# PJLab-ADG/neuralsim

Hardware: NVIDIA H100
Metric: Mrays/sec fwd+bwd (higher is better)
Workload: dtype f16

## Files before the change

### neuralsim_b200/csrc/fused_tc.cu

```cuda
#include "fused_tc_common.cuh"

namespace nsb {

constexpr int kSdfCtasPerSM = 4, kSdfPackCtasPerSM = 5;

template <int MODE>
__global__ void __launch_bounds__(kTile, MODE == 2 ? kSdfPackCtasPerSM : 0)
k_fused_sdf_tc(const PLMeta m, const __half *__restrict__ grid, const DecoderDevTC dec, const float *__restrict__ x,
               const float *__restrict__ rays_o, const float *__restrict__ rays_d, const int64_t *__restrict__ ridx,
               const float *__restrict__ t, int64_t n, int max_level, float *__restrict__ sdf, const int64_t *__restrict__ pack_infos,
               const int64_t *__restrict__ pack_ray, const int64_t *__restrict__ order, int64_t n_packs, const OccCollect oc,
               const int64_t *__restrict__ n_dev) {
    if (MODE == 2) n_packs = eff_n(n_packs, n_dev); else n = eff_n(n, n_dev);
    __shared__ __align__(128) uint8_t sA[kTile * NF * 2];
    __shared__ __align__(128) uint8_t sB[HW * NF * 2];
    __shared__ float sb1[HW], sW2[HW], srow[kTile];
    __shared__ float sb2;

    const int tid = threadIdx.x, warp = tid >> 5, lane = tid & 31;
    stage_W1(dec, sB, tid);
    stage_decoder_vectors(dec, sb1, sW2, &sb2, tid);
    tc::fence_async_smem();
    __syncthreads();
    const SdfTile ctx{m, grid, max_level, sA, tc::smem_u32(sA), tc::smem_u32(sB), srow, sb1, sW2, sb2, SoftplusK(dec.beta)};

    if (MODE == 2) {
        const int64_t n_groups = (n_packs + 31) / 32;
        for (int64_t g = blockIdx.x; g < n_groups; g += gridDim.x) {
            const int64_t slot = g * 32 + lane;
            int64_t first = 0, cnt = 0, ray = 0;
            if (slot < n_packs) {
                const int64_t p = order ? order[slot] : slot;
                first = pack_infos[2 * p]; cnt = pack_infos[2 * p + 1]; ray = pack_ray ? pack_ray[p] : p;
            }
            float o[3] = {0.f, 0.f, 0.f}, d[3] = {0.f, 0.f, 0.f};
            if (cnt > 0) {
#pragma unroll
                for (int q = 0; q < 3; ++q) { o[q] = rays_o[ray * 3 + q]; d[q] = rays_d[ray * 3 + q]; }
            }
            int max_n = (int)cnt;
#pragma unroll
            for (int s = 16; s > 0; s >>= 1) max_n = max(max_n, __shfl_xor_sync(0xffffffffu, max_n, s));
            for (int k0 = 0; k0 < max_n; k0 += kTile / 32) {
                const int k = k0 + warp;
                const bool valid = k < cnt;
                float xs[3] = {0.f, 0.f, 0.f};
                if (valid) {
                    const float tt = t[first + k];
#pragma unroll
                    for (int q = 0; q < 3; ++q) xs[q] = __fmaf_rn(d[q], tt, o[q]);
                }
#pragma unroll
                for (int q = 0; q < 3; ++q) xs[q] = to_table_space(xs[q]);
                const float v = sdf_of_tile(ctx, xs, tid);
                if (valid) {
                    sdf[first + k] = v;
                    if (oc.pcl) occ_collect_point(oc, xs, v);
                }
            }
        }
    } else {
        const int64_t n_tiles = (n + kTile - 1) / kTile;
        for (int64_t tile = blockIdx.x; tile < n_tiles; tile += gridDim.x) {
            const int64_t i = tile * kTile + tid;
            const bool valid = i < n;
            float xs[3];
            load_point(PointSrc{x, rays_o, rays_d, t, ridx}, MODE == 1, i, valid, xs);
            const float v = sdf_of_tile(ctx, xs, tid);
            if (valid) {
                sdf[i] = v;
                if (oc.pcl) occ_collect_point(oc, xs, v);
            }
        }
    }
}

constexpr int kSdfBwdCtasPerSM = 4;

template <bool FROM_RAYS, bool kXGrad>
__global__ void __launch_bounds__(kTile, kSdfBwdCtasPerSM)
k_sdf_bwd_tc(const PLMeta m, const __half *__restrict__ grid, const DecoderDevTC dec, const float *__restrict__ x,
             const float *__restrict__ rays_o, const float *__restrict__ rays_d, const int64_t *__restrict__ ridx,
             const float *__restrict__ t, const float *__restrict__ d_sdf, int64_t n, int max_level, float *__restrict__ d_grid,
             float *__restrict__ d_W1, float *__restrict__ d_b1, float *__restrict__ d_W2, float *__restrict__ d_b2,
             const int64_t *__restrict__ keep, const int64_t *__restrict__ n_dev, float *__restrict__ gx_out) {
    n = eff_n(n, n_dev);
    constexpr int NX = 40, GW = 128;
    constexpr int kS = tc::acc_stride(NF);
    extern __shared__ uint8_t dyn_smem[];
    uint8_t *tiles = reinterpret_cast<uint8_t *>((reinterpret_cast<uintptr_t>(dyn_smem) + 127) & ~uintptr_t(127));
    uint8_t *sA = tiles;
    uint8_t *sG = sA + kTile * NX * 2;
    uint8_t *sB = sG + kTile * GW * 2;
    uint8_t *sBT = sB + HW * NF * 2;
    float *stage = reinterpret_cast<float *>(sG);
    static_assert(kTile * kS * 4 <= kTile * GW * 2, "the staged dH rows must fit in G");
    __shared__ float sb1[HW], sW2[HW], sdd[kTile];
    __shared__ float sdb2;

    const int tid = threadIdx.x, lane = tid & 31;
    stage_W1(dec, sB, tid);
    stage_W1T(dec, sBT, tid);
    stage_decoder_vectors(dec, sb1, sW2, nullptr, tid);
    *reinterpret_cast<uint4 *>(sA + 4 * (kTile * 16) + tid * 16) = make_uint4(0x00003C00u, 0, 0, 0);
    float xacc[NX / 2], vacc[4];
#pragma unroll
    for (int k = 0; k < NX / 2; ++k) xacc[k] = 0.f;
#pragma unroll
    for (int k = 0; k < 4; ++k) vacc[k] = 0.f;
    if (tid == 0) sdb2 = 0.f;
    tc::fence_async_smem();
    __syncthreads();
    const uint32_t a_addr = tc::smem_u32(sA), g_addr = tc::smem_u32(sG), b_addr = tc::smem_u32(sB), bt_addr = tc::smem_u32(sBT);
    const SoftplusK spk(dec.beta);
    bool first_tile = true;

    const int64_t n_tiles = (n + kTile - 1) / kTile;
    for (int64_t tile = blockIdx.x; tile < n_tiles; tile += gridDim.x) {
        const int64_t i_ = tile * kTile + tid;
        const bool valid = i_ < n;
        const int64_t i = (valid && keep) ? keep[i_] : i_;
        float xs[3];
        load_point(PointSrc{x, rays_o, rays_d, t, ridx}, FROM_RAYS, i, valid, xs);
        const float dd = valid ? d_sdf[i] : 0.f;
        sdd[tid] = dd;
        gather_row_to_tile<kTile>(m, grid, xs, max_level, sA, tid);
        tc::fence_async_smem();
        __syncthreads();
        {
            float z[2][HW / 2];
            tc::mma_m128<HW, 0, 0, NF / 16>(z, tc::kmajor(a_addr, kTile), tc::kmajor(b_addr, HW), false);
#pragma unroll
            for (int h = 0; h < 2; ++h)
#pragma unroll
                for (int r = 0; r < 2; ++r) {
                    const int row = h * 64 + tc::frag_row(r);
                    const float d = sdd[row];
#pragma unroll
                    for (int c = 0; c < HW / 8; ++c) {
                        const int col = tc::frag_col(c);
                        float dz[2], da[2];
#pragma unroll
                        for (int j = 0; j < 2; ++j) {
                            const float zz = r16(z[h][4 * c + 2 * r + j] + sb1[col + j]);
                            float a, s;
                            softplus_as(zz, spk, a, s);
                            da[j] = d * r16(a);
                            dz[j] = d * sW2[col + j] * s;
                        }
                        tc::st_pair_f16(sG, tc::pair_off<kTile>(row, col), dz[0], dz[1]);
                        tc::st_pair_f16(sG, tc::pair_off<kTile>(row, HW + col), da[0], da[1]);
                    }
                }
        }
        tc::fence_async_smem();
        __syncthreads();
        float dh_fr[2][NF / 2];
        tc::mma_m128<NF, 0, 0, HW / 16>(dh_fr, tc::kmajor(g_addr, kTile), tc::kmajor(bt_addr, NF), false);
        tc::mma_m64<NX, 1, 1, kTile / 16>(xacc, tc::mnmajor(g_addr, kTile), tc::mnmajor(a_addr, kTile), true);
        tc::mma_m64<8, 1, 1, kTile / 16>(vacc, tc::mnmajor(g_addr + 8 * (kTile * 16), kTile), tc::mnmajor(a_addr + 4 * (kTile * 16), kTile), true);
        first_tile = false;
        const float dsum = warp_sum(dd);
        if (lane == 0 && dsum != 0.f) atomicAdd(&sdb2, dsum);
        __syncthreads();
        tc::frag_store<NF>(dh_fr, stage, kS, 0);
        __syncthreads();
        const bool active = valid && dd != 0.f;
        const bool warp_active = __any_sync(0xffffffffu, active);
        float gx[3] = {0.f, 0.f, 0.f};
#pragma unroll 1
        for (uint32_t g4 = 0; g4 * 4 < m.n_pseudo; ++g4) {
            float dh[8];
            tc::acc_ld8(stage, kS, tid, g4 * 8, dh);
            if (!warp_active) continue;
#pragma unroll
            for (uint32_t q = 0; q < 4; ++q) {
                const uint32_t p = g4 * 4 + q;
                if (p >= m.n_pseudo || (int)m.level[p] > max_level) continue;
                uint32_t cell[8];
                float w[8], a[8], b[8], fr[3], sc[3];
                if constexpr (kXGrad) level_cells3(m, p, xs, cell, w, fr, sc);
                else level_cells3(m, p, xs, cell, w);
                const float g0 = active ? dh[2 * q] : 0.f, g1 = active ? dh[2 * q + 1] : 0.f;
                if constexpr (kXGrad) level_input_grad(m, p, grid, cell, fr, sc, g0, g1, gx);
#pragma unroll
                for (int c = 0; c < 8; ++c) { a[c] = g0 * w[c]; b[c] = g1 * w[c]; }
                if (warp_merge_updates(cell_key3(m, p, xs), active, a, b, lane)) {
                    float2 *gp = level_grad_ptr(m, p, d_grid);
#pragma unroll
                    for (int c = 0; c < 8; ++c) red_add2(gp + cell[c], a[c], b[c]);
                }
            }
        }
        if constexpr (kXGrad) {
            if (valid) {
                float g[3];
#pragma unroll
                for (int d = 0; d < 3; ++d) g[d] = input_grad_to_net(gx[d]);
                const float tt = t[i];
                float4 *o = reinterpret_cast<float4 *>(gx_out + i_ * 8);
                o[0] = make_float4(g[0], g[1], g[2], __fmul_rn(tt, g[0]));
                o[1] = make_float4(__fmul_rn(tt, g[1]), __fmul_rn(tt, g[2]), 0.f, 0.f);
            }
        }
        __syncthreads();
    }
    if (!first_tile) {
#pragma unroll
        for (int r = 0; r < 2; ++r) {
            const int row = tc::frag_row(r);
            if (row >= dec.width) continue;
#pragma unroll
            for (int c = 0; c <= NF / 8; ++c)
#pragma unroll
                for (int j = 0; j < 2; ++j) {
                    const int col = tc::frag_col(c) + j;
                    if (col < dec.nh) atomicAdd(d_W1 + row * dec.nh + col, xacc[4 * c + 2 * r + j]);
                    else if (col == NF) atomicAdd(d_b1 + row, xacc[4 * c + 2 * r + j]);
                }
            if (tc::frag_col(0) == 0) atomicAdd(d_W2 + row, vacc[2 * r]);
        }
        if (tid == 0) atomicAdd(d_b2, sdb2);
    }
}

}

using namespace nsb;

extern "C" int nsb_fused_sdf_tc_launch(const nsb_lotd_meta *meta, const void *params_half, const nsb_sdf_decoder *dec, const float *x,
                                       const float *rays_o, const float *rays_d, const int64_t *ridx, const float *t, int64_t n,
                                       int32_t max_level, float *sdf, void *stream, int mode, const int64_t *pack_infos,
                                       const int64_t *pack_ray, const int64_t *pack_order, int64_t n_packs, const nsb_occ_collect *collect) {
    const DevCounts dn = take_counts();
    PLMeta m;
    DecoderDevTC d;
    if (int rc = make_decoder(meta, dec, &m, &d, "nsb_fused_sdf (tensor-core)")) return rc;
    cudaStream_t s = (cudaStream_t)stream;
    const int ml = max_level < 0 ? -1 : max_level;
    const __half *g = (const __half *)params_half;
    const OccCollect oc = occ_collect_of(collect);
    const unsigned tiles = persistent_grid((n + kTile - 1) / kTile, kSdfCtasPerSM);
    if (mode == 2 && require_ctas_per_sm(k_fused_sdf_tc<2>, kTile, 0, kSdfPackCtasPerSM, "nsb_fused_sdf (packs)")) return 2;
    if (mode == 2)
        k_fused_sdf_tc<2><<<persistent_grid((n_packs + 31) / 32, kSdfPackCtasPerSM), kTile, 0, s>>>(m, g, d, nullptr, rays_o, rays_d, nullptr, t, n, ml, sdf,
                                                                                                 pack_infos, pack_ray, pack_order, n_packs, oc, dn.a);
    else if (mode == 1)
        k_fused_sdf_tc<1><<<tiles, kTile, 0, s>>>(m, g, d, nullptr, rays_o, rays_d, ridx, t, n, ml, sdf, nullptr, nullptr, nullptr, 0, oc, dn.a);
    else
        k_fused_sdf_tc<0><<<tiles, kTile, 0, s>>>(m, g, d, x, nullptr, nullptr, nullptr, nullptr, n, ml, sdf, nullptr, nullptr, nullptr, 0, oc, dn.a);
    return check_launch("nsb_fused_sdf(tc)");
}

extern "C" int nsb_fused_sdf_bwd(const nsb_lotd_meta *meta, const void *params_half, const nsb_sdf_decoder *dec, const float *x,
                                 const float *rays_o, const float *rays_d, const int64_t *ridx, const float *t, const float *d_sdf,
                                 int64_t n, int32_t max_level, float *d_grid, float *d_W1, float *d_b1, float *d_W2, float *d_b2,
                                 void *stream) {
    return nsb_fused_sdf_bwd_indexed(meta, params_half, dec, x, rays_o, rays_d, ridx, t, d_sdf, nullptr, n, max_level, d_grid, d_W1, d_b1, d_W2, d_b2,
                                     stream);
}

template <bool kXGrad>
static int sdf_bwd(const char *who, const nsb_lotd_meta *meta, const void *params_half, const nsb_sdf_decoder *dec, const float *x, const float *rays_o,
                   const float *rays_d, const int64_t *ridx, const float *t, const float *d_sdf, const int64_t *keep, int64_t n, int32_t max_level,
                   float *d_grid, float *d_W1, float *d_b1, float *d_W2, float *d_b2, float *gx_scratch, const int64_t *ray_map, float *d_rays_o,
                   float *d_rays_d, void *stream) {
    const DevCounts dn = take_counts();
    if (n == 0) return 0;
    NSB_REQUIRE(meta && params_half && dec && d_sdf && d_grid && d_W1 && d_b1 && d_W2 && d_b2, "%s: NULL argument", who);
    NSB_REQUIRE(x || (rays_o && rays_d && t), "%s: need x or (rays_o, rays_d, t)", who);
    if (kXGrad) NSB_REQUIRE(!x && gx_scratch, "%s: ray gradients need the points as rays (x NULL) and gx_scratch", who);
    PLMeta m;
    DecoderDevTC d;
    if (int rc = make_decoder(meta, dec, &m, &d, who)) return rc;
    constexpr int kBwdSmem = (128 * 40 + 128 * 128 + 64 * 32 + 32 * 64) * 2 + 128;
    auto kern = x == nullptr ? k_sdf_bwd_tc<true, kXGrad> : k_sdf_bwd_tc<false, false>;
    opt_in_smem(kern, kBwdSmem);
    if (int rc = require_ctas_per_sm(kern, kTile, kBwdSmem, kSdfBwdCtasPerSM, who)) return rc;
    const unsigned grid = persistent_grid((n + kTile - 1) / kTile, kSdfBwdCtasPerSM);
    cudaStream_t s = (cudaStream_t)stream;
    const int ml = max_level < 0 ? -1 : max_level;
    kern<<<grid, kTile, kBwdSmem, s>>>(m, (const __half *)params_half, d, x, x ? nullptr : rays_o, x ? nullptr : rays_d, x ? nullptr : ridx,
                                       x ? nullptr : t, d_sdf, n, ml, d_grid, d_W1, d_b1, d_W2, d_b2, keep, dn.a, gx_scratch);
    if (int rc = check_launch(who)) return rc;
    if (kXGrad) {
        if (!d_rays_o && !d_rays_d) return 0;
        k_ray_row_sum<8><<<row_sum_blocks(n), 256, 0, s>>>(gx_scratch, ridx, keep, n, 6, ray_map, RowSumOut{{d_rays_o, d_rays_d, nullptr}, 3}, dn.a);
        return check_launch("nsb_fused_sdf_bwd_rays(ray sum)");
    }
    return 0;
}

extern "C" int nsb_fused_sdf_bwd_indexed(const nsb_lotd_meta *meta, const void *params_half, const nsb_sdf_decoder *dec, const float *x,
                                         const float *rays_o, const float *rays_d, const int64_t *ridx, const float *t, const float *d_sdf,
                                         const int64_t *keep, int64_t n, int32_t max_level, float *d_grid, float *d_W1, float *d_b1, float *d_W2,
                                         float *d_b2, void *stream) {
    return sdf_bwd<false>("nsb_fused_sdf_bwd", meta, params_half, dec, x, rays_o, rays_d, ridx, t, d_sdf, keep, n, max_level, d_grid, d_W1, d_b1, d_W2,
                          d_b2, nullptr, nullptr, nullptr, nullptr, stream);
}

extern "C" int nsb_fused_sdf_bwd_rays(const nsb_lotd_meta *meta, const void *params_half, const nsb_sdf_decoder *dec, const float *rays_o,
                                      const float *rays_d, const int64_t *ridx, const float *t, const float *d_sdf, const int64_t *keep, int64_t n,
                                      int32_t max_level, float *d_grid, float *d_W1, float *d_b1, float *d_W2, float *d_b2, float *gx_scratch,
                                      const int64_t *ray_map, float *d_rays_o, float *d_rays_d, void *stream) {
    return sdf_bwd<true>("nsb_fused_sdf_bwd_rays", meta, params_half, dec, nullptr, rays_o, rays_d, ridx, t, d_sdf, keep, n, max_level, d_grid, d_W1,
                         d_b1, d_W2, d_b2, gx_scratch, ray_map, d_rays_o, d_rays_d, stream);
}
```

### neuralsim_b200/csrc/fused_tc_common.cuh

```cuda
#pragma once
#include "lotd_device.cuh"
#include "tc_util.cuh"

namespace nsb {

struct DecoderDevTC {
    const __half *W1, *b1, *W2, *b2;
    int width;
    int nh;
    float beta;
};

struct OccCollect {
    float *pcl;
    int rx, ry, rz;
    float inv_s;
};
inline OccCollect occ_collect_of(const nsb_occ_collect *c) {
    if (c && c->grid_pcl) return OccCollect{c->grid_pcl, c->res[0], c->res[1], c->res[2], c->inv_s};
    return OccCollect{nullptr, 1, 1, 1, 0.f};
}
__device__ __forceinline__ float r16(float v) { return __half2float(__float2half_rn(v)); }
__device__ __forceinline__ void occ_collect_point(const OccCollect &oc, const float (&xs)[3], float sdf) {
    const int ix = min(max((int)__fmul_rn(xs[0], (float)oc.rx), 0), oc.rx - 1);
    const int iy = min(max((int)__fmul_rn(xs[1], (float)oc.ry), 0), oc.ry - 1);
    const int iz = min(max((int)__fmul_rn(xs[2], (float)oc.rz), 0), oc.rz - 1);
    const float a = fminf(fmaxf(r16(r16(__fmul_rn(sdf, oc.inv_s)) * 0.5f), -20.f), 20.f);
    const float r = r16(__fdiv_rn(1.f, r16(coshf(a))));
    const float v = r16(__fmul_rn(r, r));
    if (v > 0.f) atomicMax(reinterpret_cast<int *>(oc.pcl) + ((ix * oc.ry + iy) * oc.rz + iz), __float_as_int(v));
}

constexpr int kTile = 128;
constexpr int NF = 32, HW = 64;

template <int R>
__device__ __forceinline__ void put_level_to_tile(uint8_t *tile, int r, uint32_t p, uint32_t v) {
    *reinterpret_cast<uint32_t *>(tile + (p >> 2) * (R * 16) + r * 16 + (p & 3) * 4) = v;
}
template <int R, int U = 2>
__device__ __forceinline__ void gather_row_to_tile(const PLMeta &m, const __half *__restrict__ grid, const float (&xs)[3],
                                                   int max_level, uint8_t *tile, int r) {
    const uint32_t L = m.n_pseudo;
    uint32_t p0 = 0;
#pragma unroll 1
    for (; p0 + U <= L; p0 += U) {
        uint32_t cell[U][8];
        float w[U][8];
        uint32_t packed[U];
#pragma unroll
        for (int u = 0; u < U; ++u) level_cells3(m, p0 + u, xs, cell[u], w[u]);
#pragma unroll
        for (int u = 0; u < U; ++u) packed[u] = level_feat2_cells(level_cells_ptr(m, p0 + u, grid), cell[u], w[u]);
#pragma unroll
        for (int u = 0; u < U; ++u) {
            const uint32_t p = p0 + u;
            put_level_to_tile<R>(tile, r, p, ((int)m.level[p] <= max_level) ? packed[u] : 0u);
        }
    }
#pragma unroll 1
    for (; p0 < L; ++p0) {
        uint32_t cell[8];
        float w[8];
        level_cells3(m, p0, xs, cell, w);
        const uint32_t packed = level_feat2_cells(level_cells_ptr(m, p0, grid), cell, w);
        put_level_to_tile<R>(tile, r, p0, ((int)m.level[p0] <= max_level) ? packed : 0u);
    }
#pragma unroll 1
    for (; p0 < 16; ++p0) put_level_to_tile<R>(tile, r, p0, 0u);
}

__device__ __forceinline__ void jacobian_from_raw(const uint32_t (&raw)[8], const float (&fr)[3], const float (&scale)[3], float (&J0)[3],
                                                  float (&J1)[3]) {
    float2 v[8];
#pragma unroll
    for (int c = 0; c < 8; ++c) v[c] = __half22float2(*reinterpret_cast<const __half2 *>(&raw[c]));
#pragma unroll
    for (int gd = 0; gd < 3; ++gd) {
        float a0 = 0.f, a1 = 0.f;
#pragma unroll
        for (int c = 0; c < 4; ++c) {
            float ww = scale[gd];
            int left = 0;
#pragma unroll
            for (int k = 0; k < 2; ++k) {
                const int d = k >= gd ? k + 1 : k;
                if (c & (1 << k)) { ww = __fmul_rn(ww, fr[d]); left += 1 << d; }
                else ww = __fmul_rn(ww, __fsub_rn(1.f, fr[d]));
            }
            const int right = left + (1 << gd);
            a0 = __fmaf_rn(ww, __fsub_rn(v[right].x, v[left].x), a0);
            a1 = __fmaf_rn(ww, __fsub_rn(v[right].y, v[left].y), a1);
        }
        J0[gd] = a0;
        J1[gd] = a1;
    }
}

__device__ __forceinline__ void level_input_grad(const PLMeta &m, uint32_t p, const __half *__restrict__ grid, const uint32_t (&cell)[8],
                                                 const float (&fr)[3], const float (&sc)[3], float h0, float h1, float (&gx)[3]) {
    uint32_t raw[8];
    const uint32_t *lp = level_cells_ptr(m, p, grid);
#pragma unroll
    for (int c = 0; c < 8; ++c) raw[c] = ld_nc_u32(lp + cell[c]);
    float J0[3], J1[3];
    jacobian_from_raw(raw, fr, sc, J0, J1);
#pragma unroll
    for (int d = 0; d < 3; ++d) gx[d] = __fmaf_rn(h1, J1[d], __fmaf_rn(h0, J0[d], gx[d]));
}

__device__ __forceinline__ float input_grad_to_net(float g) { return __fmul_rn(g, 0.5f); }

struct PointSrc {
    const float *x, *rays_o, *rays_d, *t;
    const int64_t *ridx;
};

__device__ __forceinline__ void load_point(const PointSrc &ps, bool from_rays, int64_t i, bool valid, float (&xn)[3], float (&xs)[3],
                                           int64_t &ray) {
    xn[0] = xn[1] = xn[2] = 0.f;
    ray = 0;
    if (valid) {
        if (from_rays) {
            ray = ps.ridx ? ps.ridx[i] : i;
            const float tt = ps.t[i];
#pragma unroll
            for (int d = 0; d < 3; ++d) xn[d] = __fmaf_rn(ps.rays_d[ray * 3 + d], tt, ps.rays_o[ray * 3 + d]);
        } else {
#pragma unroll
            for (int d = 0; d < 3; ++d) xn[d] = ps.x[i * 3 + d];
            ray = ps.ridx ? ps.ridx[i] : i;
        }
    }
#pragma unroll
    for (int d = 0; d < 3; ++d) xs[d] = to_table_space(xn[d]);
}
__device__ __forceinline__ void load_point(const PointSrc &ps, bool from_rays, int64_t i, bool valid, float (&xs)[3]) {
    float xn[3];
    int64_t ray;
    load_point(ps, from_rays, i, valid, xn, xs, ray);
}

struct SoftplusK {
    float k, thr, out;
    float beta;
    __device__ __forceinline__ explicit SoftplusK(float b) : k(b * 1.4426950408889634f), thr(20.f * 1.4426950408889634f), out(0.6931471805599453f / b), beta(b) {}
};
__device__ __forceinline__ float ex2_approx(float x) { float r; asm("ex2.approx.ftz.f32 %0, %1;" : "=f"(r) : "f"(x)); return r; }
__device__ __forceinline__ float lg2_approx(float x) { float r; asm("lg2.approx.ftz.f32 %0, %1;" : "=f"(r) : "f"(x)); return r; }
__device__ __forceinline__ float rcp_approx(float x) { float r; asm("rcp.approx.ftz.f32 %0, %1;" : "=f"(r) : "f"(x)); return r; }

__device__ __forceinline__ float softplus_a(float zz, const SoftplusK &K) {
    const float t = zz * K.k;
    const float e = ex2_approx(t);
    const float a = lg2_approx(1.f + e) * K.out;
    return t > K.thr ? zz : a;
}
__device__ __forceinline__ void softplus_as(float zz, const SoftplusK &K, float &a, float &s) {
    const float t = zz * K.k;
    const float e = ex2_approx(t);
    const float d = 1.f + e;
    const bool lin = t > K.thr;
    a = lin ? zz : lg2_approx(d) * K.out;
    s = lin ? 1.f : e * rcp_approx(d);
}

__device__ __forceinline__ void stage_W1(const DecoderDevTC &dec, uint8_t *sB, int tid) {
    for (int e = tid; e < HW * (NF / 8); e += kTile) {
        const int j = e % HW, c = e / HW;
        __align__(16) __half q[8];
#pragma unroll
        for (int k = 0; k < 8; ++k) q[k] = (j < dec.width && c * 8 + k < dec.nh) ? dec.W1[j * dec.nh + c * 8 + k] : __float2half_rn(0.f);
        *reinterpret_cast<uint4 *>(sB + c * (HW * 16) + j * 16) = *reinterpret_cast<const uint4 *>(q);
    }
}

__device__ __forceinline__ void stage_W1T(const DecoderDevTC &dec, uint8_t *sBT, int tid) {
    for (int e = tid; e < NF * HW; e += kTile) {
        const int k = e % NF, j = e / NF;
        const __half v = (j < dec.width && k < dec.nh) ? dec.W1[j * dec.nh + k] : __float2half_rn(0.f);
        *reinterpret_cast<__half *>(sBT + (j / 8) * (NF * 16) + k * 16 + (j % 8) * 2) = v;
    }
}

template <typename B1, typename B2>
__device__ __forceinline__ void stage_decoder_vectors(const DecoderDevTC &dec, B1 sb1, float *sW2, B2 sb2, int tid) {
    constexpr bool kB1 = !std::is_same<B1, std::nullptr_t>::value, kB2 = !std::is_same<B2, std::nullptr_t>::value;
    if (tid < HW) {
        if constexpr (kB1) sb1[tid] = tid < dec.width ? __half2float(dec.b1[tid]) : 0.f;
        sW2[tid] = tid < dec.width ? __half2float(dec.W2[tid]) : 0.f;
    }
    if constexpr (kB2) {
        if (tid == 0) *sb2 = __half2float(dec.b2[0]);
    }
}

struct RowSumOut {
    float *p[3];
    int k;
};
template <int W>
__global__ void __launch_bounds__(256)
k_ray_row_sum(const float *__restrict__ rows, const int64_t *__restrict__ ridx, const int64_t *__restrict__ keep, int64_t n, int n_out,
              const int64_t *__restrict__ ray_map, const RowSumOut out, const int64_t *__restrict__ n_dev) {
    n = eff_n(n, n_dev);
    const int lane = threadIdx.x & 31;
    const int64_t n_warps = (int64_t)gridDim.x * (blockDim.x / 32);
    auto ray_of = [&](int64_t j) { return ridx[keep ? keep[j] : j]; };
    for (int64_t w = blockIdx.x * (int64_t)(blockDim.x / 32) + threadIdx.x / 32; w * 32 < n; w += n_warps) {
        const int64_t i = w * 32 + lane;
        const int64_t ray = i < n ? (ridx ? ray_of(i) : i) : -1;
        uint32_t heads = __ballot_sync(~0u, i < n && (!ridx || i == 0 || ray_of(i - 1) != ray));
        while (heads) {
            const int src = __ffs(heads) - 1;
            heads &= heads - 1;
            const int64_t r = __shfl_sync(~0u, ray, src);
            float acc[W];
#pragma unroll
            for (int k = 0; k < W; ++k) acc[k] = 0.f;
            for (int64_t base = w * 32 + src;; base += 32) {
                const int64_t j = base + lane;
                const bool same = j < n && (ridx ? ray_of(j) == r : j == base);
                const uint32_t stop = ~__ballot_sync(~0u, same);
                const int end = stop ? __ffs(stop) - 1 : 32;
                if (lane < end) {
#pragma unroll
                    for (int q = 0; q < W / 4; ++q) {
                        const float4 a = *reinterpret_cast<const float4 *>(rows + j * W + 4 * q);
                        acc[4 * q] += a.x; acc[4 * q + 1] += a.y; acc[4 * q + 2] += a.z; acc[4 * q + 3] += a.w;
                    }
                }
                if (end < 32) break;
            }
#pragma unroll
            for (int k = 0; k < W; ++k)
#pragma unroll
                for (int off = 16; off > 0; off >>= 1) acc[k] += __shfl_xor_sync(~0u, acc[k], off);
            if (lane < n_out) {
                float v = acc[0];
#pragma unroll
                for (int k = 1; k < W; ++k) v = lane == k ? acc[k] : v;
                const int which = lane / out.k;
                float *o = which == 0 ? out.p[0] : (which == 1 ? out.p[1] : out.p[2]);
                if (o) atomicAdd(o + (ray_map ? ray_map[r] : r) * out.k + (lane - which * out.k), v);
            }
        }
    }
}

inline unsigned row_sum_blocks(int64_t n) {
    const int64_t blocks = (n + 255) / 256;
    return (unsigned)(blocks < (1 << 20) ? blocks : (1 << 20));
}

inline int make_decoder(const nsb_lotd_meta *meta, const nsb_sdf_decoder *dec, PLMeta *m, DecoderDevTC *d, const char *who) {
    if (make_plmeta(meta, m)) return 2;
    NSB_REQUIRE(m->n_pseudo >= 1 && m->n_pseudo <= 16, "%s: built for 1 to 16 LoTD levels (got %u)", who, m->n_pseudo);
    NSB_REQUIRE(m->F == 2 && m->D == 3 && m->n_out == 2 * m->n_pseudo && plmeta_two_feature_cells(*m), "%s: built for L x 2 LoTD features in 3-D", who);
    NSB_REQUIRE(plmeta_cell_key_fits(*m), "%s: a level resolution exceeds %u cells per axis (the backward's merge key)", who, 1u << kCellKeyBits);
    NSB_REQUIRE(dec->width >= 1 && dec->width <= 64, "%s: decoder width must be <= 64", who);
    *d = DecoderDevTC{(const __half *)dec->W1, (const __half *)dec->b1, (const __half *)dec->W2, (const __half *)dec->b2, dec->width,
                      2 * (int)m->n_pseudo, dec->beta};
    return 0;
}

struct SdfTile {
    const PLMeta &m;
    const __half *grid;
    int max_level;
    uint8_t *sA;
    uint32_t a_addr, b_addr;
    float *srow;
    const float *sb1, *sW2;
    float sb2;
    SoftplusK spk;
};

__device__ __forceinline__ float sdf_of_tile(const SdfTile &c, const float (&xs)[3], int tid) {
    gather_row_to_tile<kTile>(c.m, c.grid, xs, c.max_level, c.sA, tid);
    tc::fence_async_smem();
    __syncthreads();
    float z[2][HW / 2];
    tc::mma_m128<HW, 0, 0, NF / 16>(z, tc::kmajor(c.a_addr, kTile), tc::kmajor(c.b_addr, HW), false);
    const int lane = tid & 31, q = lane & 3;
#pragma unroll
    for (int h = 0; h < 2; ++h)
#pragma unroll
        for (int i = 0; i < 2; ++i) {
            float out = 0.f;
#pragma unroll
            for (int ch = 0; ch < HW / 8; ++ch)
#pragma unroll
                for (int j = 0; j < 2; ++j) {
                    const int col = ch * 8 + 2 * q + j;
                    const float zz = r16(z[h][4 * ch + 2 * i + j] + c.sb1[col]);
                    out = fmaf(r16(softplus_a(zz, c.spk)), c.sW2[col], out);
                }
            out += __shfl_xor_sync(0xffffffffu, out, 1);
            out += __shfl_xor_sync(0xffffffffu, out, 2);
            if (q == 0) c.srow[h * 64 + (tid >> 5) * 16 + (lane >> 2) + 8 * i] = out;
        }
    __syncthreads();
    return r16(c.srow[tid] + c.sb2);
}

}
```

### neuralsim_b200/csrc/tc_util.cuh

```cuda
#pragma once
#include "nsb_common.cuh"

namespace nsb {
namespace tc {

__device__ __forceinline__ uint32_t smem_u32(const void *p) { return (uint32_t)__cvta_generic_to_shared(p); }

__device__ __forceinline__ uint64_t make_desc(uint32_t smem_addr, uint32_t lbo_bytes, uint32_t sbo_bytes) {
    uint64_t d = 0;
    d |= (uint64_t)((smem_addr >> 4) & 0x3FFF);
    d |= (uint64_t)((lbo_bytes >> 4) & 0x3FFF) << 16;
    d |= (uint64_t)((sbo_bytes >> 4) & 0x3FFF) << 32;
    return d;
}

struct Operand {
    uint32_t addr, lbo, sbo, kstep;
};
__device__ __forceinline__ Operand kmajor(uint32_t addr, int rows) { return Operand{addr, (uint32_t)rows * 16, 128, (uint32_t)rows * 32}; }
__device__ __forceinline__ Operand mnmajor(uint32_t addr, int rows) { return Operand{addr, 128, (uint32_t)rows * 16, 256}; }

template <int N, int TA, int TB>
struct Wgmma;
template <int TA, int TB>
struct Wgmma<8, TA, TB> {
    __device__ __forceinline__ static void mma(float (&d)[4], uint64_t a, uint64_t b, uint32_t acc) {
        asm volatile(
            "{\n\t.reg .pred p;\n\tsetp.ne.b32 p, %6, 0;\n\t"
            "wgmma.mma_async.sync.aligned.m64n8k16.f32.f16.f16 {%0, %1, %2, %3}, %4, %5, p, 1, 1, %7, %8;\n\t}\n"
            : "+f"(d[0]), "+f"(d[1]), "+f"(d[2]), "+f"(d[3])
            : "l"(a), "l"(b), "r"(acc), "n"(TA), "n"(TB));
    }
};
template <int TA, int TB>
struct Wgmma<32, TA, TB> {
    __device__ __forceinline__ static void mma(float (&d)[16], uint64_t a, uint64_t b, uint32_t acc) {
        asm volatile(
            "{\n\t.reg .pred p;\n\tsetp.ne.b32 p, %18, 0;\n\t"
            "wgmma.mma_async.sync.aligned.m64n32k16.f32.f16.f16 {%0, %1, %2, %3, %4, %5, %6, %7, %8, %9, %10, %11, %12, %13, %14, %15}, %16, %17, p, 1, 1, %19, %20;\n\t}\n"
            : "+f"(d[0]), "+f"(d[1]), "+f"(d[2]), "+f"(d[3]), "+f"(d[4]), "+f"(d[5]), "+f"(d[6]), "+f"(d[7]), "+f"(d[8]), "+f"(d[9]), "+f"(d[10]), "+f"(d[11]), "+f"(d[12]), "+f"(d[13]), "+f"(d[14]), "+f"(d[15])
            : "l"(a), "l"(b), "r"(acc), "n"(TA), "n"(TB));
    }
};
template <int TA, int TB>
struct Wgmma<40, TA, TB> {
    __device__ __forceinline__ static void mma(float (&d)[20], uint64_t a, uint64_t b, uint32_t acc) {
        asm volatile(
            "{\n\t.reg .pred p;\n\tsetp.ne.b32 p, %22, 0;\n\t"
            "wgmma.mma_async.sync.aligned.m64n40k16.f32.f16.f16 {%0, %1, %2, %3, %4, %5, %6, %7, %8, %9, %10, %11, %12, %13, %14, %15, %16, %17, %18, %19}, %20, %21, p, 1, 1, %23, %24;\n\t}\n"
            : "+f"(d[0]), "+f"(d[1]), "+f"(d[2]), "+f"(d[3]), "+f"(d[4]), "+f"(d[5]), "+f"(d[6]), "+f"(d[7]), "+f"(d[8]), "+f"(d[9]), "+f"(d[10]), "+f"(d[11]), "+f"(d[12]), "+f"(d[13]), "+f"(d[14]), "+f"(d[15]), "+f"(d[16]), "+f"(d[17]), "+f"(d[18]), "+f"(d[19])
            : "l"(a), "l"(b), "r"(acc), "n"(TA), "n"(TB));
    }
};
template <int TA, int TB>
struct Wgmma<48, TA, TB> {
    __device__ __forceinline__ static void mma(float (&d)[24], uint64_t a, uint64_t b, uint32_t acc) {
        asm volatile(
            "{\n\t.reg .pred p;\n\tsetp.ne.b32 p, %26, 0;\n\t"
            "wgmma.mma_async.sync.aligned.m64n48k16.f32.f16.f16 {%0, %1, %2, %3, %4, %5, %6, %7, %8, %9, %10, %11, %12, %13, %14, %15, %16, %17, %18, %19, %20, %21, %22, %23}, %24, %25, p, 1, 1, %27, %28;\n\t}\n"
            : "+f"(d[0]), "+f"(d[1]), "+f"(d[2]), "+f"(d[3]), "+f"(d[4]), "+f"(d[5]), "+f"(d[6]), "+f"(d[7]), "+f"(d[8]), "+f"(d[9]), "+f"(d[10]), "+f"(d[11]), "+f"(d[12]), "+f"(d[13]), "+f"(d[14]), "+f"(d[15]), "+f"(d[16]), "+f"(d[17]), "+f"(d[18]), "+f"(d[19]), "+f"(d[20]), "+f"(d[21]), "+f"(d[22]), "+f"(d[23])
            : "l"(a), "l"(b), "r"(acc), "n"(TA), "n"(TB));
    }
};
template <int TA, int TB>
struct Wgmma<64, TA, TB> {
    __device__ __forceinline__ static void mma(float (&d)[32], uint64_t a, uint64_t b, uint32_t acc) {
        asm volatile(
            "{\n\t.reg .pred p;\n\tsetp.ne.b32 p, %34, 0;\n\t"
            "wgmma.mma_async.sync.aligned.m64n64k16.f32.f16.f16 {%0, %1, %2, %3, %4, %5, %6, %7, %8, %9, %10, %11, %12, %13, %14, %15, %16, %17, %18, %19, %20, %21, %22, %23, %24, %25, %26, %27, %28, %29, %30, %31}, %32, %33, p, 1, 1, %35, %36;\n\t}\n"
            : "+f"(d[0]), "+f"(d[1]), "+f"(d[2]), "+f"(d[3]), "+f"(d[4]), "+f"(d[5]), "+f"(d[6]), "+f"(d[7]), "+f"(d[8]), "+f"(d[9]), "+f"(d[10]), "+f"(d[11]), "+f"(d[12]), "+f"(d[13]), "+f"(d[14]), "+f"(d[15]), "+f"(d[16]), "+f"(d[17]), "+f"(d[18]), "+f"(d[19]), "+f"(d[20]), "+f"(d[21]), "+f"(d[22]), "+f"(d[23]), "+f"(d[24]), "+f"(d[25]), "+f"(d[26]), "+f"(d[27]), "+f"(d[28]), "+f"(d[29]), "+f"(d[30]), "+f"(d[31])
            : "l"(a), "l"(b), "r"(acc), "n"(TA), "n"(TB));
    }
};
template <int TA, int TB>
struct Wgmma<80, TA, TB> {
    __device__ __forceinline__ static void mma(float (&d)[40], uint64_t a, uint64_t b, uint32_t acc) {
        asm volatile(
            "{\n\t.reg .pred p;\n\tsetp.ne.b32 p, %42, 0;\n\t"
            "wgmma.mma_async.sync.aligned.m64n80k16.f32.f16.f16 {%0, %1, %2, %3, %4, %5, %6, %7, %8, %9, %10, %11, %12, %13, %14, %15, %16, %17, %18, %19, %20, %21, %22, %23, %24, %25, %26, %27, %28, %29, %30, %31, %32, %33, %34, %35, %36, %37, %38, %39}, %40, %41, p, 1, 1, %43, %44;\n\t}\n"
            : "+f"(d[0]), "+f"(d[1]), "+f"(d[2]), "+f"(d[3]), "+f"(d[4]), "+f"(d[5]), "+f"(d[6]), "+f"(d[7]), "+f"(d[8]), "+f"(d[9]), "+f"(d[10]), "+f"(d[11]), "+f"(d[12]), "+f"(d[13]), "+f"(d[14]), "+f"(d[15]), "+f"(d[16]), "+f"(d[17]), "+f"(d[18]), "+f"(d[19]), "+f"(d[20]), "+f"(d[21]), "+f"(d[22]), "+f"(d[23]), "+f"(d[24]), "+f"(d[25]), "+f"(d[26]), "+f"(d[27]), "+f"(d[28]), "+f"(d[29]), "+f"(d[30]), "+f"(d[31]), "+f"(d[32]), "+f"(d[33]), "+f"(d[34]), "+f"(d[35]), "+f"(d[36]), "+f"(d[37]), "+f"(d[38]), "+f"(d[39])
            : "l"(a), "l"(b), "r"(acc), "n"(TA), "n"(TB));
    }
};

__device__ __forceinline__ void wgmma_fence() { asm volatile("wgmma.fence.sync.aligned;" ::: "memory"); }
__device__ __forceinline__ void wgmma_commit() { asm volatile("wgmma.commit_group.sync.aligned;" ::: "memory"); }
__device__ __forceinline__ void wgmma_wait_all() { asm volatile("wgmma.wait_group.sync.aligned 0;" ::: "memory"); }
__device__ __forceinline__ void fence_operand(float &r) { asm volatile("" : "+f"(r)::"memory"); }

template <int N, int TA, int TB, int KSTEPS>
__device__ __forceinline__ void mma_m128(float (&d)[2][N / 2], const Operand &a, const Operand &b, bool accumulate) {
#pragma unroll
    for (int h = 0; h < 2; ++h)
#pragma unroll
        for (int i = 0; i < N / 2; ++i) fence_operand(d[h][i]);
    wgmma_fence();
#pragma unroll
    for (int h = 0; h < 2; ++h)
#pragma unroll
        for (int ks = 0; ks < KSTEPS; ++ks)
            Wgmma<N, TA, TB>::mma(d[h], make_desc(a.addr + h * 8 * a.sbo + ks * a.kstep, a.lbo, a.sbo), make_desc(b.addr + ks * b.kstep, b.lbo, b.sbo),
                                  (ks > 0 || accumulate) ? 1u : 0u);
    wgmma_commit();
    wgmma_wait_all();
#pragma unroll
    for (int h = 0; h < 2; ++h)
#pragma unroll
        for (int i = 0; i < N / 2; ++i) fence_operand(d[h][i]);
}

template <int N, int TA, int TB, int KSTEPS>
__device__ __forceinline__ void mma_m64(float (&d)[N / 2], const Operand &a, const Operand &b, bool accumulate) {
#pragma unroll
    for (int i = 0; i < N / 2; ++i) fence_operand(d[i]);
    wgmma_fence();
#pragma unroll
    for (int ks = 0; ks < KSTEPS; ++ks)
        Wgmma<N, TA, TB>::mma(d, make_desc(a.addr + ks * a.kstep, a.lbo, a.sbo), make_desc(b.addr + ks * b.kstep, b.lbo, b.sbo),
                              (ks > 0 || accumulate) ? 1u : 0u);
    wgmma_commit();
    wgmma_wait_all();
#pragma unroll
    for (int i = 0; i < N / 2; ++i) fence_operand(d[i]);
}

__device__ __forceinline__ int frag_row(int i) { return (threadIdx.x >> 5) * 16 + ((threadIdx.x & 31) >> 2) + 8 * i; }
__device__ __forceinline__ int frag_col(int c) { return c * 8 + 2 * (threadIdx.x & 3); }
template <int R>
__device__ __forceinline__ uint32_t pair_off(int row, int col) { return (uint32_t)((col >> 3) * (R * 16) + row * 16 + (col & 7) * 2); }
__device__ __forceinline__ float2 ld_pair_f16(const uint8_t *tile, uint32_t off) {
    return __half22float2(*reinterpret_cast<const __half2 *>(tile + off));
}
__device__ __forceinline__ void st_pair_f16(uint8_t *tile, uint32_t off, float a, float b) {
    *reinterpret_cast<__half2 *>(tile + off) = __floats2half2_rn(a, b);
}

constexpr int acc_stride(int cols) { return cols + 4; }

template <int N>
__device__ __forceinline__ void frag_store(const float (&d)[2][N / 2], float *acc, int stride, int col0) {
    const int w = threadIdx.x >> 5, l = threadIdx.x & 31;
#pragma unroll
    for (int h = 0; h < 2; ++h)
#pragma unroll
        for (int c = 0; c < N / 8; ++c)
#pragma unroll
            for (int i = 0; i < 2; ++i) {
                const int row = h * 64 + w * 16 + (l >> 2) + 8 * i, col = col0 + c * 8 + 2 * (l & 3);
                *reinterpret_cast<float2 *>(acc + row * stride + col) = make_float2(d[h][4 * c + 2 * i], d[h][4 * c + 2 * i + 1]);
            }
}
template <int N>
__device__ __forceinline__ void frag_load(float (&d)[2][N / 2], const float *acc, int stride, int col0) {
    const int w = threadIdx.x >> 5, l = threadIdx.x & 31;
#pragma unroll
    for (int h = 0; h < 2; ++h)
#pragma unroll
        for (int c = 0; c < N / 8; ++c)
#pragma unroll
            for (int i = 0; i < 2; ++i) {
                const int row = h * 64 + w * 16 + (l >> 2) + 8 * i, col = col0 + c * 8 + 2 * (l & 3);
                const float2 v = *reinterpret_cast<const float2 *>(acc + row * stride + col);
                d[h][4 * c + 2 * i] = v.x;
                d[h][4 * c + 2 * i + 1] = v.y;
            }
}
template <int N, int TA, int TB, int KSTEPS>
__device__ __forceinline__ void mma_to_rows(float *acc, int stride, int col0, const Operand &a, const Operand &b, bool accumulate) {
    float d[2][N / 2];
    if (accumulate) frag_load<N>(d, acc, stride, col0);
    else {
#pragma unroll
        for (int h = 0; h < 2; ++h)
#pragma unroll
            for (int i = 0; i < N / 2; ++i) d[h][i] = 0.f;
    }
    mma_m128<N, TA, TB, KSTEPS>(d, a, b, accumulate);
    frag_store<N>(d, acc, stride, col0);
}

__device__ __forceinline__ void acc_ld8(const float *acc, int stride, int row, int col, float (&v)[8]) {
    const float4 a = *reinterpret_cast<const float4 *>(acc + row * stride + col), b = *reinterpret_cast<const float4 *>(acc + row * stride + col + 4);
    v[0] = a.x; v[1] = a.y; v[2] = a.z; v[3] = a.w; v[4] = b.x; v[5] = b.y; v[6] = b.z; v[7] = b.w;
}

__device__ __forceinline__ void mbar_init(uint64_t *bar, uint32_t count) {
    asm volatile("mbarrier.init.shared::cta.b64 [%0], %1;" ::"r"(smem_u32(bar)), "r"(count) : "memory");
}
__device__ __forceinline__ void mbar_wait(uint64_t *bar, uint32_t parity) {
    asm volatile(
        "{\n\t.reg .pred p;\n\tWAIT_%=:\n\t"
        "mbarrier.try_wait.parity.shared::cta.b64 p, [%0], %1;\n\t"
        "@p bra DONE_%=;\n\tbra WAIT_%=;\n\tDONE_%=:\n\t}\n" ::"r"(smem_u32(bar)),
        "r"(parity)
        : "memory");
}

__device__ __forceinline__ void mbar_arrive_expect_tx(uint64_t *bar, uint32_t bytes) {
    asm volatile("mbarrier.arrive.expect_tx.shared::cta.b64 _, [%0], %1;" ::"r"(smem_u32(bar)), "r"(bytes) : "memory");
}
__device__ __forceinline__ void tma_load_bulk(void *smem_dst, const void *gmem_src, uint32_t bytes, uint64_t *bar) {
    uint64_t pol;
    asm volatile("createpolicy.fractional.L2::evict_first.b64 %0, 1.0;" : "=l"(pol));
    asm volatile("cp.async.bulk.shared::cluster.global.mbarrier::complete_tx::bytes.L2::cache_hint [%0], [%1], %2, [%3], %4;"
                 ::"r"(smem_u32(smem_dst)), "l"(gmem_src), "r"(bytes), "r"(smem_u32(bar)), "l"(pol)
                 : "memory");
}

__device__ __forceinline__ void fence_async_smem() { asm volatile("fence.proxy.async.shared::cta;" ::: "memory"); }
__device__ __forceinline__ void fence_mbar_init() { asm volatile("fence.mbarrier_init.release.cluster;" ::: "memory"); }

__device__ __forceinline__ uint4 pack8_f16(const float (&v)[8]) {
    __half2 h0 = __floats2half2_rn(v[0], v[1]), h1 = __floats2half2_rn(v[2], v[3]);
    __half2 h2 = __floats2half2_rn(v[4], v[5]), h3 = __floats2half2_rn(v[6], v[7]);
    uint4 q;
    q.x = *reinterpret_cast<uint32_t *>(&h0); q.y = *reinterpret_cast<uint32_t *>(&h1);
    q.z = *reinterpret_cast<uint32_t *>(&h2); q.w = *reinterpret_cast<uint32_t *>(&h3);
    return q;
}

template <int R, int K>
__device__ __forceinline__ void store_row_f16(uint8_t *tile, int r, const float *vals) {
#pragma unroll
    for (int c = 0; c < K / 8; ++c) {
        __half2 h0 = __floats2half2_rn(vals[c * 8 + 0], vals[c * 8 + 1]);
        __half2 h1 = __floats2half2_rn(vals[c * 8 + 2], vals[c * 8 + 3]);
        __half2 h2 = __floats2half2_rn(vals[c * 8 + 4], vals[c * 8 + 5]);
        __half2 h3 = __floats2half2_rn(vals[c * 8 + 6], vals[c * 8 + 7]);
        uint4 q;
        q.x = *reinterpret_cast<uint32_t *>(&h0);
        q.y = *reinterpret_cast<uint32_t *>(&h1);
        q.z = *reinterpret_cast<uint32_t *>(&h2);
        q.w = *reinterpret_cast<uint32_t *>(&h3);
        *reinterpret_cast<uint4 *>(tile + c * (R * 16) + r * 16) = q;
    }
}

}
}
```

Measured before the change: 30.95.

## Warp-specialize packed SDF forward into gather producers and wgmma consumer ring

The packed-ray SDF forward kernel becomes one large CTA per SM. Five producer warpgroups gather hash-grid features into a ring of seven shared-memory tiles, and one consumer warpgroup runs the wgmma MLP and writes outputs, with mbarriers handing tiles between them. Register budgets are rebalanced with setmaxnreg. The goal is to overlap memory-bound feature gathering with tensor-core work and remove the per-tile __syncthreads of the old single-warpgroup design. The risks are a consumer bottleneck, lower CTA-level occupancy, and more synchronisation complexity.

New measurement: 32.65, median of 6. 1.05x the previous value.

```diff
diff --git a/neuralsim_b200/csrc/fused_tc.cu b/neuralsim_b200/csrc/fused_tc.cu
--- a/neuralsim_b200/csrc/fused_tc.cu
+++ b/neuralsim_b200/csrc/fused_tc.cu
@@ -2,64 +2,163 @@
 
 namespace nsb {
 
-constexpr int kSdfCtasPerSM = 4, kSdfPackCtasPerSM = 5;
+constexpr int kSdfCtasPerSM = 4;
+
+constexpr int kPackSets = 5, kPackSlots = 7, kPackCtasPerSM = 1;
+constexpr int kPackProducerRegs = 72, kPackConsumerRegs = 120;
+static_assert(kPackSets * kTile * kPackProducerRegs + kTile * kPackConsumerRegs <= kTile * (1 + kPackSets) * 80, "register split");
+constexpr int kPackThreads = kTile * (1 + kPackSets);
+constexpr int kPackSmem = kPackSlots * (kTile * NF * 2 + kTile * 12) + HW * NF * 2 + 2 * HW * 4 + kPackSlots * 20 + 16 + 128;
+
+struct PackSlots {
+    uint8_t *a;
+    int64_t *out;
+    int *voxel;
+    uint64_t *full, *empty;
+    int *end;
+};
+
+__device__ __forceinline__ void sdf_packs_produce(const PLMeta &m, const __half *__restrict__ grid, int max_level, const float *__restrict__ rays_o,
+                                                  const float *__restrict__ rays_d, const float *__restrict__ t, const int64_t *__restrict__ pack_infos,
+                                                  const int64_t *__restrict__ pack_ray, const int64_t *__restrict__ order, int64_t n_packs,
+                                                  const OccCollect &oc, const PackSlots &ring, int set, int w, int lane) {
+    const int row = w * 32 + lane;
+    const int64_t n_groups = (n_packs + 31) / 32;
+    uint32_t j = 0;
+    for (int64_t g = blockIdx.x; g < n_groups; g += gridDim.x) {
+        const int64_t slot = g * 32 + lane;
+        int64_t first = 0, cnt = 0, ray = 0;
+        if (slot < n_packs) {
+            const int64_t p = order ? order[slot] : slot;
+            first = pack_infos[2 * p]; cnt = pack_infos[2 * p + 1]; ray = pack_ray ? pack_ray[p] : p;
+        }
+        int max_n = (int)cnt;
+#pragma unroll
+        for (int s = 16; s > 0; s >>= 1) max_n = max(max_n, __shfl_xor_sync(0xffffffffu, max_n, s));
+        const uint32_t tiles = (uint32_t)(max_n + 3) / 4;
+        uint32_t mine = j + (uint32_t)((set - (int)(j % kPackSets) + kPackSets) % kPackSets);
+        if (mine < j + tiles) {
+            float o[3] = {0.f, 0.f, 0.f}, d[3] = {0.f, 0.f, 0.f};
+            if (cnt > 0) {
+#pragma unroll
+                for (int q = 0; q < 3; ++q) { o[q] = rays_o[ray * 3 + q]; d[q] = rays_d[ray * 3 + q]; }
+            }
+            for (; mine < j + tiles; mine += kPackSets) {
+                const int k = (int)(mine - j) * 4 + w;
+                const bool valid = k < cnt;
+                float xs[3] = {0.f, 0.f, 0.f};
+                if (valid) {
+                    const float tt = t[first + k];
+#pragma unroll
+                    for (int q = 0; q < 3; ++q) xs[q] = __fmaf_rn(d[q], tt, o[q]);
+                }
+#pragma unroll
+                for (int q = 0; q < 3; ++q) xs[q] = to_table_space(xs[q]);
+                const uint32_t s = mine % kPackSlots;
+                tc::mbar_wait(&ring.empty[s], ((mine / kPackSlots) & 1u) ^ 1u);
+                gather_row_to_tile<kTile>(m, grid, xs, max_level, ring.a + s * (kTile * NF * 2), row);
+                ring.out[s * kTile + row] = valid ? first + k : -1;
+                ring.voxel[s * kTile + row] = (valid && oc.pcl) ? occ_voxel(oc, xs) : 0;
+                tc::fence_async_smem();
+                tc::mbar_arrive(&ring.full[s]);
+            }
+        }
+        j += tiles;
+    }
+    if ((int)(j % kPackSets) == set) {
+        const uint32_t s = j % kPackSlots;
+        tc::mbar_wait(&ring.empty[s], ((j / kPackSlots) & 1u) ^ 1u);
+        if (row == 0) ring.end[s] = 1;
+        tc::mbar_arrive(&ring.full[s]);
+    }
+}
 
 template <int MODE>
-__global__ void __launch_bounds__(kTile, MODE == 2 ? kSdfPackCtasPerSM : 0)
+__global__ void __launch_bounds__(MODE == 2 ? kPackThreads : kTile, MODE == 2 ? kPackCtasPerSM : 0)
 k_fused_sdf_tc(const PLMeta m, const __half *__restrict__ grid, const DecoderDevTC dec, const float *__restrict__ x,
                const float *__restrict__ rays_o, const float *__restrict__ rays_d, const int64_t *__restrict__ ridx,
                const float *__restrict__ t, int64_t n, int max_level, float *__restrict__ sdf, const int64_t *__restrict__ pack_infos,
                const int64_t *__restrict__ pack_ray, const int64_t *__restrict__ order, int64_t n_packs, const OccCollect oc,
                const int64_t *__restrict__ n_dev) {
-    if (MODE == 2) n_packs = eff_n(n_packs, n_dev); else n = eff_n(n, n_dev);
-    __shared__ __align__(128) uint8_t sA[kTile * NF * 2];
-    __shared__ __align__(128) uint8_t sB[HW * NF * 2];
-    __shared__ float sb1[HW], sW2[HW], srow[kTile];
-    __shared__ float sb2;
-
-    const int tid = threadIdx.x, warp = tid >> 5, lane = tid & 31;
-    stage_W1(dec, sB, tid);
-    stage_decoder_vectors(dec, sb1, sW2, &sb2, tid);
-    tc::fence_async_smem();
-    __syncthreads();
-    const SdfTile ctx{m, grid, max_level, sA, tc::smem_u32(sA), tc::smem_u32(sB), srow, sb1, sW2, sb2, SoftplusK(dec.beta)};
-
-    if (MODE == 2) {
-        const int64_t n_groups = (n_packs + 31) / 32;
-        for (int64_t g = blockIdx.x; g < n_groups; g += gridDim.x) {
-            const int64_t slot = g * 32 + lane;
-            int64_t first = 0, cnt = 0, ray = 0;
-            if (slot < n_packs) {
-                const int64_t p = order ? order[slot] : slot;
-                first = pack_infos[2 * p]; cnt = pack_infos[2 * p + 1]; ray = pack_ray ? pack_ray[p] : p;
-            }
-            float o[3] = {0.f, 0.f, 0.f}, d[3] = {0.f, 0.f, 0.f};
-            if (cnt > 0) {
-#pragma unroll
-                for (int q = 0; q < 3; ++q) { o[q] = rays_o[ray * 3 + q]; d[q] = rays_d[ray * 3 + q]; }
-            }
-            int max_n = (int)cnt;
-#pragma unroll
-            for (int s = 16; s > 0; s >>= 1) max_n = max(max_n, __shfl_xor_sync(0xffffffffu, max_n, s));
-            for (int k0 = 0; k0 < max_n; k0 += kTile / 32) {
-                const int k = k0 + warp;
-                const bool valid = k < cnt;
-                float xs[3] = {0.f, 0.f, 0.f};
-                if (valid) {
-                    const float tt = t[first + k];
-#pragma unroll
-                    for (int q = 0; q < 3; ++q) xs[q] = __fmaf_rn(d[q], tt, o[q]);
+    const int tid = threadIdx.x;
+    if constexpr (MODE == 2) {
+        const int warp = tid >> 5, lane = tid & 31;
+        n_packs = eff_n(n_packs, n_dev);
+        extern __shared__ uint8_t dyn_smem[];
+        uint8_t *base = reinterpret_cast<uint8_t *>((reinterpret_cast<uintptr_t>(dyn_smem) + 127) & ~uintptr_t(127));
+        PackSlots ring;
+        ring.a = base;
+        uint8_t *sB = ring.a + kPackSlots * (kTile * NF * 2);
+        ring.out = reinterpret_cast<int64_t *>(sB + HW * NF * 2);
+        ring.voxel = reinterpret_cast<int *>(ring.out + kPackSlots * kTile);
+        float *sb1 = reinterpret_cast<float *>(ring.voxel + kPackSlots * kTile), *sW2 = sb1 + HW;
+        ring.full = reinterpret_cast<uint64_t *>(sW2 + HW);
+        ring.empty = ring.full + kPackSlots;
+        ring.end = reinterpret_cast<int *>(ring.empty + kPackSlots);
+        float *sb2 = reinterpret_cast<float *>(ring.end + kPackSlots);
+        if (tid < kTile) {
+            stage_W1(dec, sB, tid);
+            stage_decoder_vectors(dec, sb1, sW2, sb2, tid);
+        }
+        if (tid < kPackSlots) {
+            tc::mbar_init(&ring.full[tid], kTile);
+            tc::mbar_init(&ring.empty[tid], kTile);
+            ring.end[tid] = 0;
+        }
+        tc::fence_mbar_init();
+        tc::fence_async_smem();
+        __syncthreads();
+        if (warp >= 4) {
+            tc::setmaxnreg_dec<kPackProducerRegs>();
+            sdf_packs_produce(m, grid, max_level, rays_o, rays_d, t, pack_infos, pack_ray, order, n_packs, oc, ring, (warp - 4) >> 2, warp & 3, lane);
+            return;
+        }
+        tc::setmaxnreg_inc<kPackConsumerRegs>();
+        const uint32_t b_addr = tc::smem_u32(sB);
+        const SoftplusK spk(dec.beta);
+        const float b2 = *sb2;
+        for (uint32_t j = 0;; ++j) {
+            const uint32_t s = j % kPackSlots;
+            tc::mbar_wait(&ring.full[s], (j / kPackSlots) & 1u);
+            if (ring.end[s]) break;
+            float z[2][HW / 2];
+            tc::mma_m128<HW, 0, 0, NF / 16>(z, tc::kmajor(tc::smem_u32(ring.a + s * (kTile * NF * 2)), kTile), tc::kmajor(b_addr, HW), false);
+            int64_t out_i[2][2];
+            int vox[2][2];
+#pragma unroll
+            for (int h = 0; h < 2; ++h)
+#pragma unroll
+                for (int i = 0; i < 2; ++i) {
+                    const int row = h * 64 + tc::frag_row(i);
+                    out_i[h][i] = ring.out[s * kTile + row];
+                    vox[h][i] = ring.voxel[s * kTile + row];
                 }
-#pragma unroll
-                for (int q = 0; q < 3; ++q) xs[q] = to_table_space(xs[q]);
-                const float v = sdf_of_tile(ctx, xs, tid);
-                if (valid) {
-                    sdf[first + k] = v;
-                    if (oc.pcl) occ_collect_point(oc, xs, v);
-                }
+            tc::mbar_arrive(&ring.empty[s]);
+            float v[2][2];
+            sdf_rows_of_frags(z, sb1, sW2, spk, v);
+            if ((lane & 3) == 0) {
+#pragma unroll
+                for (int h = 0; h < 2; ++h)
+#pragma unroll
+                    for (int i = 0; i < 2; ++i) {
+                        if (out_i[h][i] < 0) continue;
+                        const float r = r16(v[h][i] + b2);
+                        sdf[out_i[h][i]] = r;
+                        if (oc.pcl) occ_collect_voxel(oc, vox[h][i], r);
+                    }
             }
         }
     } else {
+        n = eff_n(n, n_dev);
+        __shared__ __align__(128) uint8_t sA[kTile * NF * 2];
+        __shared__ __align__(128) uint8_t sB[HW * NF * 2];
+        __shared__ float sb1[HW], sW2[HW], srow[kTile];
+        __shared__ float sb2;
+        stage_W1(dec, sB, tid);
+        stage_decoder_vectors(dec, sb1, sW2, &sb2, tid);
+        tc::fence_async_smem();
+        __syncthreads();
+        const SdfTile ctx{m, grid, max_level, sA, tc::smem_u32(sA), tc::smem_u32(sB), srow, sb1, sW2, sb2, SoftplusK(dec.beta)};
         const int64_t n_tiles = (n + kTile - 1) / kTile;
         for (int64_t tile = blockIdx.x; tile < n_tiles; tile += gridDim.x) {
             const int64_t i = tile * kTile + tid;
@@ -241,11 +340,12 @@
     const __half *g = (const __half *)params_half;
     const OccCollect oc = occ_collect_of(collect);
     const unsigned tiles = persistent_grid((n + kTile - 1) / kTile, kSdfCtasPerSM);
-    if (mode == 2 && require_ctas_per_sm(k_fused_sdf_tc<2>, kTile, 0, kSdfPackCtasPerSM, "nsb_fused_sdf (packs)")) return 2;
-    if (mode == 2)
-        k_fused_sdf_tc<2><<<persistent_grid((n_packs + 31) / 32, kSdfPackCtasPerSM), kTile, 0, s>>>(m, g, d, nullptr, rays_o, rays_d, nullptr, t, n, ml, sdf,
-                                                                                                 pack_infos, pack_ray, pack_order, n_packs, oc, dn.a);
-    else if (mode == 1)
+    if (mode == 2) {
+        opt_in_smem(k_fused_sdf_tc<2>, kPackSmem);
+        if (int rc = require_ctas_per_sm(k_fused_sdf_tc<2>, kPackThreads, kPackSmem, kPackCtasPerSM, "nsb_fused_sdf (packs)")) return rc;
+        k_fused_sdf_tc<2><<<persistent_grid((n_packs + 31) / 32, kPackCtasPerSM), kPackThreads, kPackSmem, s>>>(
+            m, g, d, nullptr, rays_o, rays_d, nullptr, t, n, ml, sdf, pack_infos, pack_ray, pack_order, n_packs, oc, dn.a);
+    } else if (mode == 1)
         k_fused_sdf_tc<1><<<tiles, kTile, 0, s>>>(m, g, d, nullptr, rays_o, rays_d, ridx, t, n, ml, sdf, nullptr, nullptr, nullptr, 0, oc, dn.a);
     else
         k_fused_sdf_tc<0><<<tiles, kTile, 0, s>>>(m, g, d, x, nullptr, nullptr, nullptr, nullptr, n, ml, sdf, nullptr, nullptr, nullptr, 0, oc, dn.a);
diff --git a/neuralsim_b200/csrc/fused_tc_common.cuh b/neuralsim_b200/csrc/fused_tc_common.cuh
--- a/neuralsim_b200/csrc/fused_tc_common.cuh
+++ b/neuralsim_b200/csrc/fused_tc_common.cuh
@@ -21,14 +21,20 @@
     return OccCollect{nullptr, 1, 1, 1, 0.f};
 }
 __device__ __forceinline__ float r16(float v) { return __half2float(__float2half_rn(v)); }
-__device__ __forceinline__ void occ_collect_point(const OccCollect &oc, const float (&xs)[3], float sdf) {
+__device__ __forceinline__ int occ_voxel(const OccCollect &oc, const float (&xs)[3]) {
     const int ix = min(max((int)__fmul_rn(xs[0], (float)oc.rx), 0), oc.rx - 1);
     const int iy = min(max((int)__fmul_rn(xs[1], (float)oc.ry), 0), oc.ry - 1);
     const int iz = min(max((int)__fmul_rn(xs[2], (float)oc.rz), 0), oc.rz - 1);
+    return (ix * oc.ry + iy) * oc.rz + iz;
+}
+__device__ __forceinline__ void occ_collect_voxel(const OccCollect &oc, int voxel, float sdf) {
     const float a = fminf(fmaxf(r16(r16(__fmul_rn(sdf, oc.inv_s)) * 0.5f), -20.f), 20.f);
     const float r = r16(__fdiv_rn(1.f, r16(coshf(a))));
     const float v = r16(__fmul_rn(r, r));
-    if (v > 0.f) atomicMax(reinterpret_cast<int *>(oc.pcl) + ((ix * oc.ry + iy) * oc.rz + iz), __float_as_int(v));
+    if (v > 0.f) atomicMax(reinterpret_cast<int *>(oc.pcl) + voxel, __float_as_int(v));
+}
+__device__ __forceinline__ void occ_collect_point(const OccCollect &oc, const float (&xs)[3], float sdf) {
+    occ_collect_voxel(oc, occ_voxel(oc, xs), sdf);
 }
 
 constexpr int kTile = 128;
@@ -276,30 +282,42 @@
     SoftplusK spk;
 };
 
+__device__ __forceinline__ void sdf_rows_of_frags(const float (&z)[2][HW / 2], const float *sb1, const float *sW2, const SoftplusK &spk,
+                                                  float (&out)[2][2]) {
+    const int q = threadIdx.x & 3;
+#pragma unroll
+    for (int h = 0; h < 2; ++h)
+#pragma unroll
+        for (int i = 0; i < 2; ++i) {
+            float o = 0.f;
+#pragma unroll
+            for (int ch = 0; ch < HW / 8; ++ch)
+#pragma unroll
+                for (int j = 0; j < 2; ++j) {
+                    const int col = ch * 8 + 2 * q + j;
+                    const float zz = r16(z[h][4 * ch + 2 * i + j] + sb1[col]);
+                    o = fmaf(r16(softplus_a(zz, spk)), sW2[col], o);
+                }
+            o += __shfl_xor_sync(0xffffffffu, o, 1);
+            o += __shfl_xor_sync(0xffffffffu, o, 2);
+            out[h][i] = o;
+        }
+}
+
 __device__ __forceinline__ float sdf_of_tile(const SdfTile &c, const float (&xs)[3], int tid) {
     gather_row_to_tile<kTile>(c.m, c.grid, xs, c.max_level, c.sA, tid);
     tc::fence_async_smem();
     __syncthreads();
     float z[2][HW / 2];
     tc::mma_m128<HW, 0, 0, NF / 16>(z, tc::kmajor(c.a_addr, kTile), tc::kmajor(c.b_addr, HW), false);
-    const int lane = tid & 31, q = lane & 3;
-#pragma unroll
-    for (int h = 0; h < 2; ++h)
-#pragma unroll
-        for (int i = 0; i < 2; ++i) {
-            float out = 0.f;
-#pragma unroll
-            for (int ch = 0; ch < HW / 8; ++ch)
-#pragma unroll
-                for (int j = 0; j < 2; ++j) {
-                    const int col = ch * 8 + 2 * q + j;
-                    const float zz = r16(z[h][4 * ch + 2 * i + j] + c.sb1[col]);
-                    out = fmaf(r16(softplus_a(zz, c.spk)), c.sW2[col], out);
-                }
-            out += __shfl_xor_sync(0xffffffffu, out, 1);
-            out += __shfl_xor_sync(0xffffffffu, out, 2);
-            if (q == 0) c.srow[h * 64 + (tid >> 5) * 16 + (lane >> 2) + 8 * i] = out;
-        }
+    float out[2][2];
+    sdf_rows_of_frags(z, c.sb1, c.sW2, c.spk, out);
+    if ((tid & 3) == 0) {
+#pragma unroll
+        for (int h = 0; h < 2; ++h)
+#pragma unroll
+            for (int i = 0; i < 2; ++i) c.srow[h * 64 + tc::frag_row(i)] = out[h][i];
+    }
     __syncthreads();
     return r16(c.srow[tid] + c.sb2);
 }
diff --git a/neuralsim_b200/csrc/tc_util.cuh b/neuralsim_b200/csrc/tc_util.cuh
--- a/neuralsim_b200/csrc/tc_util.cuh
+++ b/neuralsim_b200/csrc/tc_util.cuh
@@ -186,6 +186,9 @@
 
 __device__ __forceinline__ void mbar_init(uint64_t *bar, uint32_t count) {
     asm volatile("mbarrier.init.shared::cta.b64 [%0], %1;" ::"r"(smem_u32(bar)), "r"(count) : "memory");
+}
+__device__ __forceinline__ void mbar_arrive(uint64_t *bar) {
+    asm volatile("mbarrier.arrive.shared::cta.b64 _, [%0];" ::"r"(smem_u32(bar)) : "memory");
 }
 __device__ __forceinline__ void mbar_wait(uint64_t *bar, uint32_t parity) {
     asm volatile(
@@ -206,6 +209,11 @@
                  ::"r"(smem_u32(smem_dst)), "l"(gmem_src), "r"(bytes), "r"(smem_u32(bar)), "l"(pol)
                  : "memory");
 }
+
+template <int N>
+__device__ __forceinline__ void setmaxnreg_dec() { asm volatile("setmaxnreg.dec.sync.aligned.u32 %0;" ::"n"(N)); }
+template <int N>
+__device__ __forceinline__ void setmaxnreg_inc() { asm volatile("setmaxnreg.inc.sync.aligned.u32 %0;" ::"n"(N)); }
 
 __device__ __forceinline__ void fence_async_smem() { asm volatile("fence.proxy.async.shared::cta;" ::: "memory"); }
 __device__ __forceinline__ void fence_mbar_init() { asm volatile("fence.mbarrier_init.release.cluster;" ::: "memory"); }
```
